# OverLordGoldDragon/ssqueezepy

Measured on AMD Instinct MI355X. Metric: ssq_cwt transforms/sec (N=160k, 300 scales, f32), higher is better.
Workload: dtype f32; 1 GPU; ssq_cwt('gmw'), N=160000, 300 log scales (nv=32), float32, two-chirp+noise; algo=blockzoom+tiles, tile_kernel=float64 tile, unordered ds_add_f64, column pair per lane (tile3_kernel)

## Files before the change

ssqueezepy_amd/csrc/ssq_blocks.h:

```cpp
#pragma once
#include "ssq_common.h"
#include "ssq_fft.h"
#include "ssq_tiles.h"
#include <algorithm>
#include <vector>

namespace ssq {

struct BlockRowDev {
    int32_t cls;
    int32_t klo;
    int32_t KP;
    int32_t L;
    int32_t G;
    int32_t pb_off;
};

struct BlockClassDev {
    int64_t P, m, V, nb;
    int64_t ctw_off;
    int64_t xb_off;
    int64_t blk_off;
    int64_t xb_stride;
    int64_t analytic;
};

struct BlockPlan {
    int64_t M = 0, N = 0, n1 = 0, na = 0, max_batch = 1;
    int dtype = SSQ_F32;
    int group = 1;
    int ncu = 256;
    int nc = 0;
    DeviceArena mem;
    std::vector<BlockClassDev> hcls;
    BlockClassDev* classes = nullptr;
    BlockRowDev* rows = nullptr;
    void* pbank = nullptr;
    void* pxi = nullptr;
    void* ctw = nullptr; void* ftw = nullptr;
    void* items[5] = {nullptr, nullptr, nullptr, nullptr, nullptr};
    std::vector<int32_t> h_items[5];
    int64_t n_items[5] = {0, 0, 0, 0, 0};
    int64_t ftw_off[5] = {0, 0, 0, 0, 0};
    void* blocks = nullptr;
    void* xb = nullptr;
    std::vector<FftPlan> ffts;
    std::vector<int> fft_first;
    void* xa = nullptr;
    FftPlan inv_m;
    AnalyticFft* ana = nullptr;
    int n_analytic = 0;
    bool own4096 = false;
    bool own_big = false;
    bool paired = true;
    int64_t n_generic = 0;
    bool exact_ok = false;
    int exA = 0, exB = 0, n_exact = 0;
    void* twM = nullptr; void* zbuf = nullptr;
    const float* e_bank = nullptr; const int64_t* e_off = nullptr; const int32_t* e_lo = nullptr;
    const int32_t* e_rows = nullptr;
    int setup_exact(const float* bank_dev, const int64_t* band_off_dev, const int32_t* band_lo_dev,
                    const int32_t* gen_rows_dev, const std::vector<int64_t>& h_off,
                    const std::vector<int32_t>& h_lo, const std::vector<int32_t>& h_gen);
    int run_exact(int sig, int nsig, const void* xh_all, float* Wx, float* dWx, float* w, unsigned short* kidx,
                  const float* row_scale, double dt, const SsqParams& sp, hipStream_t stream);

    int create(const ssq_cwt_blocks_desc& d, int dtype, int64_t M, int64_t N, int64_t n1, int64_t na,
               int64_t max_batch);
    void destroy();
    int64_t bytes() const;
    int spectra(const void* xp, const void* xh, int64_t batch, hipStream_t stream,
                const unsigned char* need = nullptr);
    int run(int sig, int nsig, float* Wx, float* dWx, float* w, unsigned short* kidx,
            const float* row_scale, double dt, const SsqParams& sp, hipStream_t stream,
            const int64_t* limit = nullptr);
    int run64(int sig, int nsig, double* Wx, double* dWx, double* w, unsigned short* kidx,
              const double* row_scale, double dt, const SsqParams& sp, hipStream_t stream);
};

}
```

ssqueezepy_amd/csrc/ssq_cwt_blocks.hip:

```cpp
#include "ssq_common.h"
#include "ssq_blocks.h"
#include "ssq_ldsfft.h"
#include <cmath>

namespace ssq {

#include "ssq_point_math.inl"

struct EmitRow {
    float2* W; float2* D; float* w; unsigned short* k;
    float rs; bool scale; double gamma; int64_t omax;
    float m2hi, m2lo;
    int fx, fa;
};
__device__ __forceinline__ EmitRow make_emit_row(float* Wx, float* dWx, float* w, unsigned short* kidx,
                                                 const float* row_scale, int sig, int ksig, int row,
                                                 int64_t na, int64_t N, double gamma, int flipud) {
    EmitRow e;
    const int64_t base = ((int64_t)sig * na + row) * N;
    e.W = reinterpret_cast<float2*>(Wx) + base;
    e.D = dWx ? reinterpret_cast<float2*>(dWx) + base : nullptr;
    e.w = w ? w + base : nullptr;
    e.k = kidx ? kidx + (int64_t)ksig * na * N + kidx_index(row, 0, na, N) : nullptr;
    e.scale = row_scale != nullptr;
// ... 2 lines not shown
    const float g2 = (float)(gamma * gamma);
    e.m2hi = g2 * 1.000004f; e.m2lo = g2 * 0.999996f;
    e.fx = flipud ? -1 : 0; e.fa = flipud ? (int)na : 0;
    return e;
}
template <bool LEAN, int GRID>
__device__ __forceinline__ bool emit_point(const EmitRow& e, int j, c32 W, c32 D, const SsqParams& sp) {
    float c = W.x, d = W.y, a = D.x, b = D.y;
    if constexpr (LEAN) {
        e.W[(unsigned)j] = make_float2(c, d);
        const float m2 = c * c + d * d, num = b * c - a * d;
        const bool above = m2 > e.m2hi, below = m2 < e.m2lo;
        const float w32 = fabsf(num * __builtin_amdgcn_rcpf(m2 * 6.2831855f));
        bool ok;
        const int kb = bin_screen_cwt<GRID>(w32, sp, (int)e.omax, ok);
        const int kf = (kb ^ e.fx) + e.fa;
        e.k[(unsigned)j] = (unsigned short)(above ? kf : 0xFFFF);
        return !(below | (above & ok));
    } else {
        c = c * e.rs; d = d * e.rs; a = a * e.rs; b = b * e.rs;
        e.W[j] = make_float2(c, d);
        if (e.D) e.D[j] = make_float2(a, b);
        if (e.w) {
            float wv;
            if (mag_lt(c, d, (float)e.gamma)) wv = INFINITY;
            else wv = (float)fabs(phase_ratio(a, b, c, d));
            e.w[j] = wv;
        }
        if (e.k) {
            const int above = mag_gt_screen(c, d, e.gamma);
            if (above < 0) return true;
            unsigned short kk = 0xFFFFu;
            if (above) {
                const int kb = bin_of_point_screen(a, b, c, d, sp, (int)e.omax);
                if (kb == -2) return true;
                kk = (unsigned short)(sp.flipud ? (int)e.omax - kb : kb);
            }
            e.k[j] = kk;
        }
        return false;
    }
}
template <int V> struct GridTag { static constexpr int value = V; };
template <bool LEAN, typename F>
__device__ __forceinline__ void dispatch_grid(int grid, F&& f) {
    if constexpr (LEAN) {
        if (grid == SSQ_GRID_LOG) f(GridTag<SSQ_GRID_LOG>{});
        else if (grid == SSQ_GRID_LOG_PIECEWISE) f(GridTag<SSQ_GRID_LOG_PIECEWISE>{});
        else f(GridTag<SSQ_GRID_LIN>{});
    } else {
        f(GridTag<-1>{});
    }
}
__device__ __forceinline__ void emit_point_exact(const EmitRow& e, unsigned short* kout, c32 W, c32 D,
                                                 const SsqParams& sp) {
    const float c = W.x * e.rs, d = W.y * e.rs, a = D.x * e.rs, b = D.y * e.rs;
    unsigned short kk = 0xFFFFu;
    if (mag_of(c, d) > e.gamma) {
        const int64_t kb = bin_of_point_exact(a, b, c, d, sp, e.omax);
        kk = (unsigned short)(sp.flipud ? e.omax - kb : kb);
    }
    *kout = kk;
}
struct BlockArgs {
    const int4* items;
    const BlockRowDev* rows;
    const BlockClassDev* classes;
    const float* pbank;
    const float* pxi;
    const c32* ctw;
    const c32* ftw;
    const c32* xb;
    const float* row_scale;
    float* Wx; float* dWx; float* w; unsigned short* kidx;
    int64_t M, N, na, n_items;
    double h;
    float inv_dt;
    double gamma;
    int sig;
    bool lean() const { return kidx && !dWx && !w && !row_scale; }
    bool wx_alone() const { return !kidx && !dWx && !w; }
};

template <int L, bool LEAN, bool NOD = false, bool PAIRED = true>
__device__ __forceinline__ void blockzoom_body(const BlockArgs& A, const SsqParams& sp, int item_idx,
                                               c32* __restrict__ buf, c32* __restrict__ spow,
                                               c32* __restrict__ wrapf, c32* __restrict__ bandW,
                                               c32* __restrict__ bandD) {
    using S = FftShape<L>;
    constexpr int G = S::G, R1 = S::R1, RL = S::RL;
    const int tid = threadIdx.x;
    const int4 item = A.items[item_idx];
    const int row = item.x, blk = item.y, c0 = item.z;
    const BlockRowDev r = A.rows[row];
    const BlockClassDev cl = A.classes[item.w];
    const int P = (int)cl.P, Rp = P / L;
    const int sig = A.sig + (int)blockIdx.y;
    const c32* xb = A.xb + cl.xb_off + ((int64_t)sig * cl.nb + blk) * cl.xb_stride;
    const c32* ctw = A.ctw + cl.ctw_off;
    const float* psi = A.pbank + r.pb_off;
    const float* pxi = A.pxi + r.pb_off;

    constexpr bool STAGE = (L <= 512);
    const float invP = 1.0f / (float)P;
    constexpr bool EARLY = !STAGE && (R1 * G <= NT);
    float e_p[EARLY ? PPT : 1], e_m[EARLY ? PPT : 1];
    c32 e_X[EARLY ? PPT : 1], e_cw[EARLY ? PPT / R1 : 1];
    if constexpr (EARLY) {
        constexpr int NBe = PPT / R1, STR = L / R1;
        c32 st_v = {0.f, 0.f}, st_w = {0.f, 0.f};
        if (tid < R1 * G) {
            const unsigned t = (unsigned)(tid / G), col = (unsigned)(c0 + tid % G);
            st_v = ctw[(t * (unsigned)STR * col) & (unsigned)(P - 1)];
        }
        if (tid < G) st_w = ctw[(0u - (unsigned)L * (unsigned)(c0 + tid)) & (unsigned)(P - 1)];
#pragma unroll
        for (int it = 0; it < NBe; ++it) {
            const int idx = tid + it * NT, g = idx % G, u = idx / G;
            const int off0 = (u - r.klo) & (L - 1);
            e_cw[it] = ctw[((unsigned)(r.klo + off0) * (unsigned)(c0 + g)) & (unsigned)(P - 1)];
#pragma unroll
            for (int k = 0; k < R1; ++k) {
                const int off = (off0 + k * STR) & (L - 1);
                const bool in = off < r.KP;
                e_p[it * R1 + k] = in ? psi[off] : 0.f;
                e_X[it * R1 + k] = in ? xb[r.klo + off] : c32{0.f, 0.f};
                e_m[it * R1 + k] = in ? pxi[off] : 0.f;
            }
        }
        if (tid < R1 * G) spow[tid] = st_v;
        if (tid < G) wrapf[tid] = st_w;
    } else {
        constexpr int STR = L / R1;
        for (int i = tid; i < R1 * G; i += NT) {
            const unsigned t = (unsigned)(i / G), col = (unsigned)(c0 + i % G);
            spow[i] = ctw[(t * (unsigned)STR * col) & (unsigned)(P - 1)];
        }
        if (tid < G) {
            const unsigned col = (unsigned)(c0 + tid);
            wrapf[tid] = ctw[(0u - (unsigned)L * col) & (unsigned)(P - 1)];
        }
        if constexpr (STAGE) {
            for (int off = tid; off < L; off += NT) {
                c32 b = {0.f, 0.f}, d = {0.f, 0.f};
                if (off < r.KP) {
                    const float p = psi[off] * invP;
                    const c32 X = xb[r.klo + off];
                    b = {p * X.x, p * X.y};
                    const float mm = pxi[off] * A.inv_dt;
                    d = {-(b.y * mm), b.x * mm};
                }
                bandW[off] = b; bandD[off] = d;
            }
        }
    }
    __syncthreads();
    c32 zw[PPT], zd[PPT];
    {
        constexpr int NB = PPT / R1, STR = L / R1;
#pragma unroll
        for (int it = 0; it < NB; ++it) {
            const int idx = tid + it * NT, g = idx % G, u = idx / G;
            const unsigned col = (unsigned)(c0 + g);
            const int off0 = (u - r.klo) & (L - 1);
            const c32 cw0 = EARLY ? e_cw[EARLY ? it : 0] : ctw[((unsigned)(r.klo + off0) * col) & (unsigned)(P - 1)];
            const c32 wf = wrapf[g];
#pragma unroll
            for (int k = 0; k < R1; ++k) {
                const int offu = off0 + k * STR;
                const int off = offu & (L - 1);
                c32 z = {0.f, 0.f}, dz = {0.f, 0.f};
                if constexpr (STAGE) {
                    c32 cw = (k == 0) ? cw0 : cmul_v(cw0, spow[k * G + g]);
                    if (offu >= L) cw = cmul_v(cw, wf);
                    z = cmul_v(bandW[off], cw);
                    dz = cmul_v(bandD[off], cw);
                } else if (EARLY || off < r.KP) {
                    const float p = (EARLY ? e_p[EARLY ? it * R1 + k : 0] : psi[off]) * invP;
                    const c32 X = EARLY ? e_X[EARLY ? it * R1 + k : 0] : xb[r.klo + off];
                    c32 cw = (k == 0) ? cw0 : cmul_v(cw0, spow[k * G + g]);
                    if (offu >= L) cw = cmul_v(cw, wf);
                    const c32 bz = {p * X.x, p * X.y};
                    z = cmul_v(bz, cw);
                    const float mm = (EARLY ? e_m[EARLY ? it * R1 + k : 0] : pxi[off]) * A.inv_dt;
                    dz = {-(z.y * mm), z.x * mm};
                }
                zw[it * R1 + k] = z; zd[it * R1 + k] = dz;
            }
        }
    }
    if constexpr (PAIRED && !NOD) {
        lds_ifft2<L>(zw, zd, buf, A.ftw, tid);
    } else {
        lds_ifft<L, true, true>(zw, buf, A.ftw, tid);
        if constexpr (!NOD) lds_ifft<L, true>(zd, buf, A.ftw, tid);
    }

    constexpr int NB = PPT / RL, STR = L / RL;
    const EmitRow er = make_emit_row(A.Wx, A.dWx, A.w, A.kidx, A.row_scale, sig, (int)blockIdx.y, row, A.na, A.N, A.gamma, sp.flipud);
    const int m = (int)cl.m, N = (int)A.N;
    const int jbase = blk * (int)cl.V - m + c0;
    const unsigned span = (unsigned)max(0, min((int)cl.V, N - blk * (int)cl.V));
    unsigned pend = 0;
    auto emit_all = [&](auto grid_tag) {
        constexpr int GRID = decltype(grid_tag)::value;
#pragma unroll
        for (int it = 0; it < NB; ++it) {
            const int idx = tid + it * NT, g = idx % G, u = idx / G;
#pragma unroll
            for (int k = 0; k < RL; ++k) {
                const int dcol = (u + k * STR) * Rp + g + (c0 - m);
                if ((unsigned)dcol >= span) continue;
                const int j = dcol + blk * (int)cl.V;
                if constexpr (NOD) {
                    er.W[j] = make_float2(zw[it * RL + k].x * er.rs, zw[it * RL + k].y * er.rs);
                    continue;
                }
                if (emit_point<LEAN, GRID>(er, j, zw[it * RL + k], NOD ? c32{0.f, 0.f} : zd[it * RL + k], sp))
                    pend |= 1u << (it * RL + k);
            }
        }
    };
    dispatch_grid<LEAN>(sp.grid, emit_all);
    while (__builtin_amdgcn_ballot_w64(pend != 0)) {
        const unsigned low = pend & (0u - pend);
        pend ^= low;
        c32 W = {0.f, 0.f}, D = {0.f, 0.f};
        int j = 0;
#pragma unroll
        for (int it = 0; it < NB; ++it) {
            const int idx = tid + it * NT, g = idx % G, u = idx / G;
#pragma unroll
            for (int k = 0; k < RL; ++k)
                if (low == (1u << (it * RL + k))) {
                    W = zw[it * RL + k]; D = NOD ? c32{0.f, 0.f} : zd[it * RL + k]; j = jbase + (u + k * STR) * Rp + g;
                }
        }
        if (low) emit_point_exact(er, er.k + j, W, D, sp);
    }
}

template <int L, bool LEAN, bool NOD = false, bool PAIRED = true>
__global__ __launch_bounds__(NT) void blockzoom_kernel(BlockArgs A, SsqParams sp) {
    __shared__ c32 buf[(PAIRED && !NOD) ? lds_ifft2_points<L> : D_POINTS];
    __shared__ c32 spow[FftShape<L>::R1 * FftShape<L>::G];
    __shared__ c32 wrapf[FftShape<L>::G];
    __shared__ c32 bandW[(L <= 512) ? L : 1], bandD[(L <= 512) ? L : 1];
    blockzoom_body<L, LEAN, NOD, PAIRED>(A, sp, (int)blockIdx.x, buf, spow, wrapf, bandW, bandD);
}

struct BlockMultiArgs {
    BlockArgs A;
    const int4* items[5]; const c32* ftw[5];
    int first[6];
};
template <bool LEAN, bool NOD = false, bool PAIRED = true>
__global__ __launch_bounds__(NT) void blockzoom_multi_kernel(BlockMultiArgs M, SsqParams sp) {
    __shared__ c32 buf[(PAIRED && !NOD) ? lds_ifft2_points<2048> : D_POINTS];
    __shared__ c32 spow[512];
    __shared__ c32 wrapf[32];
    __shared__ c32 bandW[512], bandD[512];
    const int b = (int)blockIdx.x;
    int s = 0;
#pragma unroll
    for (int k = 1; k < 5; ++k) s += b >= M.first[k];
    BlockArgs A = M.A;
    A.items = M.items[s]; A.ftw = M.ftw[s];
    const int it = b - M.first[s];
    switch (s) {
        case 0: blockzoom_body<128, LEAN, NOD, PAIRED>(A, sp, it, buf, spow, wrapf, bandW, bandD); break;
        case 1: blockzoom_body<256, LEAN, NOD, PAIRED>(A, sp, it, buf, spow, wrapf, bandW, bandD); break;
        case 2: blockzoom_body<512, LEAN, NOD, PAIRED>(A, sp, it, buf, spow, wrapf, bandW, bandD); break;
        case 3: blockzoom_body<1024, LEAN, NOD, PAIRED>(A, sp, it, buf, spow, wrapf, bandW, bandD); break;
        default: blockzoom_body<2048, LEAN, NOD, PAIRED>(A, sp, it, buf, spow, wrapf, bandW, bandD); break;
    }
}

struct BlockArgs64 {
    const int4* items; const BlockRowDev* rows; const BlockClassDev* classes;
    const double* pbank; const double* pxi;
    const c64* ctw; const c64* ftw; const c64* xb;
    const double* row_scale;
    double* Wx; double* dWx; double* w; unsigned short* kidx;
    int64_t M, N, na, n_items;
    double inv_dt, gamma;
    int sig;
    bool wx_alone() const { return !kidx && !dWx && !w; }
};

template <int L, bool NOD = false>
__global__ __launch_bounds__(FftGeom<double>::NT) SSQ_WAVES_PER_EU(2, 2) void blockzoom_f64_kernel(BlockArgs64 A, SsqParams sp) {
    using S = FftShape<L, double>;
    constexpr int NT64 = FftGeom<double>::NT, G = S::G, R1 = S::R1, RL = S::RL;
    __shared__ c64 buf[FftGeom<double>::D];
    __shared__ c64 spow[R1 * G];
    __shared__ c64 wrapf[G];
    const int tid = threadIdx.x;
    const int4 item = A.items[blockIdx.x];
    const int row = item.x, blk = item.y, c0 = item.z;
    const BlockRowDev r = A.rows[row];
    const BlockClassDev cl = A.classes[item.w];
    const int P = (int)cl.P, Rp = P / L;
    const int sig = A.sig + (int)blockIdx.y;
    const c64* xb = A.xb + cl.xb_off + ((int64_t)sig * cl.nb + blk) * cl.xb_stride;
    const c64* ctw = A.ctw + cl.ctw_off;
    const double* psi = A.pbank + r.pb_off;
    const double* pxi = A.pxi + r.pb_off;
    const double invP = 1.0 / (double)P;
    constexpr int NBP = PPT / R1, STRP = L / R1;
    double bp[PPT], bm[PPT]; c64 bX[PPT];
#pragma unroll
    for (int it = 0; it < NBP; ++it) {
        const int u = (tid + it * NT64) / G;
        const int off0 = (u - r.klo) & (L - 1);
#pragma unroll
        for (int k = 0; k < R1; ++k) {
            const int off = (off0 + k * STRP) & (L - 1);
            const int oc = off < r.KP ? off : 0;
            bp[it * R1 + k] = psi[oc]; bX[it * R1 + k] = xb[r.klo + oc]; bm[it * R1 + k] = pxi[oc];
        }
    }
    {
        constexpr int STR = L / R1;
        for (int i = tid; i < R1 * G; i += NT64) {
            const unsigned t = (unsigned)(i / G), col = (unsigned)(c0 + i % G);
            spow[i] = ctw[(t * (unsigned)STR * col) & (unsigned)(P - 1)];
        }
        if (tid < G) {
            const unsigned col = (unsigned)(c0 + tid);
            wrapf[tid] = ctw[(0u - (unsigned)L * col) & (unsigned)(P - 1)];
        }
    }
    c64 cw0s[NBP];
#pragma unroll
    for (int it = 0; it < NBP; ++it) {
        const int idx = tid + it * NT64, g = idx % G, u = idx / G;
        const int off0 = (u - r.klo) & (L - 1);
        cw0s[it] = ctw[((unsigned)(r.klo + off0) * (unsigned)(c0 + g)) & (unsigned)(P - 1)];
    }
    __syncthreads();
    c64 zw[PPT], zd[PPT];
    {
        constexpr int NB = PPT / R1, STR = L / R1;
#pragma unroll
        for (int it = 0; it < NB; ++it) {
            const int idx = tid + it * NT64, g = idx % G, u = idx / G;
            const int off0 = (u - r.klo) & (L - 1);
            const c64 cw0 = cw0s[it];
            const c64 wf = wrapf[g];
#pragma unroll
            for (int k = 0; k < R1; ++k) {
                const int offu = off0 + k * STR, off = offu & (L - 1);
                const bool in = off < r.KP;
                const double p = bp[it * R1 + k] * invP;
                const c64 X = bX[it * R1 + k];
                const double mm = bm[it * R1 + k] * A.inv_dt;
                c64 cw = (k == 0) ? cw0 : cmul(cw0, spow[k * G + g]);
// ... 365 lines not shown
                                                   c32* __restrict__ stw) {
    constexpr int L = WIDE_L, P = L * C, NTH = 64 * CW, SL = CW / C;
    const int tid = threadIdx.x;
    const int g = tid % CW, u = tid / CW, slot = g / C, r = g % C;
    const int64_t sig = blockIdx.y, M = A.M;
    const bool ana = k.analytic != 0;
    const int nunits = ana ? (int)k.nb : ((int)k.nb + 1) / 2;
    const c32* __restrict__ tw = A.ctw + k.ctw_off;
    const c32* __restrict__ xa = A.xa + sig * M;
    const float* __restrict__ xp = A.xp + sig * M;
    const int64_t lead = A.n1 - k.m;
    const int m32 = (int)M;
    wide_stage_tw<CW, C>(stw, tw, tid);
    c32 w[PPT / C][C];
    wide_load_w<CW, C>(w, tw, tid);
    c32 z[PPT];
    {
        const int unit = b * SL + slot;
        const bool live = unit < nunits;
        const int b0 = ana ? unit : 2 * unit, b1 = b0 + 1;
        const bool two = !ana && b1 < (int)k.nb;
        int64_t o0 = (lead + (int64_t)b0 * k.V) % M; if (o0 < 0) o0 += M;
        int64_t o1 = (lead + (int64_t)b1 * k.V) % M; if (o1 < 0) o1 += M;
        const int a0 = (int)o0, a1 = (int)o1;
#pragma unroll
        for (int t = 0; t < PPT; ++t) {
            const int p = (u + t * (L / 16)) * C + r;
            int s0 = a0 + p; if (s0 >= m32) s0 -= m32;
            int s1 = a1 + p; if (s1 >= m32) s1 -= m32;
            c32 v = {0.f, 0.f};
            if (live) {
                if (ana) v = xa[s0];
                else v = {xp[s0], two ? xp[s1] : 0.f};
            }
            z[t] = v;
        }
    }
    wide_ifft<CW>(z, buf, stw, tid);
    wide_natural<CW, C>(z, buf, w, tid);
    for (int sl = 0; sl < SL; ++sl) {
        const int unit = b * SL + sl;
        if (unit >= nunits) break;
        const int b0 = ana ? unit : 2 * unit;
        const bool two = !ana && b0 + 1 < (int)k.nb;
        const c32* __restrict__ Y = buf + sl * P;
        c32* out0 = A.xb + k.xb_off + (sig * k.nb + b0) * k.xb_stride;
        if (ana) {
            for (int f = tid; f < P; f += NTH) out0[f] = Y[(P - f) & (P - 1)];
        } else {
            c32* out1 = out0 + k.xb_stride;
            for (int f = tid; f <= P / 2; f += NTH) {
                const c32 Pk = Y[f], Qk = Y[(P - f) & (P - 1)];
                out0[f] = {0.5f * (Qk.x + Pk.x), 0.5f * (Qk.y - Pk.y)};
                if (two) out1[f] = {0.5f * (Qk.y + Pk.y), 0.5f * (Pk.x - Qk.x)};
            }
        }
    }
}
template <int QMAX>
__global__ __launch_bounds__(NT * QMAX) void block_spectra_multi_kernel(BlockSpecArgs A) {
    __shared__ c32 buf[4096 * QMAX];
    __shared__ c32 stw[WIDE_L];
    int b = (int)blockIdx.x, c = 0;
    while (c + 1 < A.ncls && b >= A.first[c + 1]) ++c;
    b -= A.first[c];
    const BlockClassDev k = A.classes[A.cls[c]];
    if (k.P == A.M && k.nb == 1 && !k.analytic && A.xh) {
        const int64_t M = A.M, sig = blockIdx.y;
        int64_t o = (A.n1 - k.m) % M; if (o < 0) o += M;
        const c32* __restrict__ tw = A.ctw + k.ctw_off;
        const c32* __restrict__ xh = A.xh + sig * (M / 2 + 1);
        c32* __restrict__ out0 = A.xb + k.xb_off + sig * k.nb * k.xb_stride;
        const unsigned mask = (unsigned)M - 1u, ou = (unsigned)o;
        for (int f = (int)threadIdx.x; f <= (int)(M / 2); f += NT * QMAX)
            out0[f] = cmul_v(xh[f], tw[((unsigned)f * ou) & mask]);
        return;
    }
    if (k.P == 4096) block_spectra_wide<4 * QMAX, 4>(A, k, b, buf, stw);
    else if (k.P == 8192) block_spectra_wide<4 * QMAX, 8>(A, k, b, buf, stw);
    else if constexpr (QMAX >= 4) block_spectra_wide<4 * QMAX, 16>(A, k, b, buf, stw);
}

template <int L>
static int launch_zoom(const BlockArgs& A, const SsqParams& sp, int nsig, bool paired, hipStream_t stream) {
    if (A.n_items == 0) return 0;
    const dim3 grid((unsigned)A.n_items, (unsigned)nsig);
    if (A.wx_alone())
        hipLaunchKernelGGL((blockzoom_kernel<L, false, true>), grid, dim3(NT), 0, stream, A, sp);
    else if (A.lean() && paired)
        hipLaunchKernelGGL((blockzoom_kernel<L, true>), grid, dim3(NT), 0, stream, A, sp);
    else if (A.lean())
        hipLaunchKernelGGL((blockzoom_kernel<L, true, false, false>), grid, dim3(NT), 0, stream, A, sp);
    else if (paired)
        hipLaunchKernelGGL((blockzoom_kernel<L, false>), grid, dim3(NT), 0, stream, A, sp);
    else
        hipLaunchKernelGGL((blockzoom_kernel<L, false, false, false>), grid, dim3(NT), 0, stream, A, sp);
    SSQ_LAUNCH_CHECK();
    return 0;
}

int BlockPlan::create(const ssq_cwt_blocks_desc& d, int dtype_, int64_t M_, int64_t N_, int64_t n1_,
                      int64_t na_, int64_t max_batch_) {
    M = M_; N = N_; n1 = n1_; na = na_; max_batch = max_batch_; dtype = dtype_;
    const size_t rs = dtype == SSQ_F32 ? 4 : 8;
    nc = d.n_classes;
    hcls.resize(nc);
    int64_t xb_total = 0, blk_max = 0;
    for (int c = 0; c < nc; ++c) {
        BlockClassDev& k = hcls[c];
        k.P = d.classes[5 * c]; k.m = d.classes[5 * c + 1]; k.V = d.classes[5 * c + 2];
        k.nb = d.classes[5 * c + 3];
        k.analytic = d.classes[5 * c + 4] ? 1 : 0;
        SSQ_REQUIRE(c == 0 || hcls[c - 1].analytic <= k.analytic, "block classes: analytic classes must come last");
        k.ctw_off = d.ctw_off[c];
        k.xb_stride = k.analytic ? k.P : k.P / 2 + 1;
        k.xb_off = xb_total;
        xb_total += max_batch * k.nb * k.xb_stride;
        k.blk_off = blk_max;
        if (!k.analytic) blk_max += max_batch * k.nb * k.P;
        n_analytic += (int)k.analytic;
    }
    int rc;
    if ((rc = mem.upload(&classes, hcls.data(), sizeof(BlockClassDev) * nc))) return rc;
    static_assert(sizeof(BlockRowDev) == 6 * sizeof(int32_t), "row table layout");
    if ((rc = mem.upload(&rows, d.rows, sizeof(BlockRowDev) * na))) return rc;
    if ((rc = mem.upload(&pbank, d.pbank, rs * d.n_pbank))) return rc;
    if ((rc = mem.upload(&pxi, d.pxi, rs * d.n_pbank))) return rc;
    if ((rc = mem.upload(&ctw, d.ctw, 2 * rs * (size_t)d.ctw_off[nc]))) return rc;
    if ((rc = mem.upload(&ftw, d.ftw, 2 * rs * (size_t)d.n_ftw))) return rc;
    for (int s = 0; s < 5; ++s) {
        n_items[s] = d.n_items[s];
        ftw_off[s] = d.ftw_off[s];
        if ((rc = mem.upload(&items[s], d.items[s], sizeof(int4) * (size_t)d.n_items[s]))) return rc;
        if (d.n_items[s]) h_items[s].assign(d.items[s], d.items[s] + 4 * d.n_items[s]);
    }
    if ((rc = mem.alloc(&xb, 2 * rs * (size_t)xb_total))) return rc;
    if ((rc = mem.alloc(&blocks, rs * (size_t)blk_max))) return rc;
    for (int c = 0; c < nc;) {
        int e = c;
        int64_t nblocks = 0;
        while (e < nc && hcls[e].P == hcls[c].P && hcls[e].analytic == hcls[c].analytic)
            nblocks += max_batch * hcls[e++].nb;
        FftPlan fp;
        rc = fp.create(hcls[c].analytic ? 2 : 0, dtype, (size_t)hcls[c].P, (size_t)nblocks, 1.0);
        if (rc) { fp.destroy(); return rc; }
        ffts.push_back(fp); fft_first.push_back(c);
        c = e;
    }
    if (n_analytic) {
        if ((rc = mem.alloc(&xa, 2 * rs * (size_t)(max_batch * M)))) return rc;
        if (AnalyticFft::supports(dtype, M)) {
            ana = new AnalyticFft();
            if ((rc = ana->create(M, max_batch))) return rc;
        } else {
            rc = inv_m.create(1, dtype, (size_t)M, (size_t)max_batch, 1.0 / (double)M);
            if (rc) return rc;
        }
    }
    n_generic = d.n_generic;
    own4096 = dtype == SSQ_F32 && M > 4096 && !(getenv("SSQ_DEBUG_BLOCK_SPECTRA") && !strcmp(getenv("SSQ_DEBUG_BLOCK_SPECTRA"), "rocfft"));
    own_big = own4096 && !(getenv("SSQ_DEBUG_BLOCK_SPECTRA") && !strcmp(getenv("SSQ_DEBUG_BLOCK_SPECTRA"), "4096"));
    paired = !(getenv("SSQ_DEBUG_BLOCK_PAIRED") && atoi(getenv("SSQ_DEBUG_BLOCK_PAIRED")) == 0);
    {
        int dev = 0; hipDeviceProp_t pr;
        bool lds128 = false;
        if (hipGetDevice(&dev) == hipSuccess && hipGetDeviceProperties(&pr, dev) == hipSuccess && pr.multiProcessorCount > 0) {
            ncu = pr.multiProcessorCount;
            lds128 = (size_t)pr.maxSharedMemoryPerMultiProcessor >= 128 * 1024;
        }
        own_big = own_big && lds128;
    }
    return 0;
}

void BlockPlan::destroy() {
    for (auto& f : ffts) f.destroy();
    inv_m.destroy();
    if (ana) { ana->destroy(); delete ana; ana = nullptr; }
    mem.release();
}

int64_t BlockPlan::bytes() const {
    int64_t b = mem.bytes() + (int64_t)inv_m.work_bytes + (ana ? ana->mem.bytes() : 0);
    for (const FftPlan& f : ffts) b += (int64_t)f.work_bytes;
    return b;
}

int BlockPlan::spectra(const void* xp, const void* xh, int64_t batch, hipStream_t stream,
                       const unsigned char* need) {
    (void)batch;
    std::vector<char> run_on(ffts.size(), 1);
    int lo[2] = {nc, nc}, hi[2] = {-1, -1};
    bool any_analytic = false;
    BlockSpecArgs S;
    S.ncls = 0; S.first[0] = 0;
    int qmax = 1;
    bool prefix[2] = {true, true};
    for (size_t f = 0; f < ffts.size(); ++f) {
        const int a = fft_first[f], b = f + 1 < ffts.size() ? fft_first[f + 1] : nc;
        bool on = !need;
        for (int c = a; c < b && !on; ++c) on = need[c] != 0;
        const int kind = (int)hcls[a].analytic;
        any_analytic = any_analytic || (on && kind);
        int wanted = 0;
        int64_t group_wgs = 0;
        for (int c = a; c < b; ++c) {
            if (need && !need[c]) continue;
            ++wanted;
            group_wgs += kind ? hcls[c].nb : (hcls[c].nb + 1) / 2;
        }
        const int64_t Pg = hcls[a].P;
        bool whole = Pg == M && !kind && xh;
        for (int c = a; c < b && whole; ++c) whole = hcls[c].nb == 1;
        const bool small = own_big && M < ((int64_t)1 << 30) && group_wgs * max_batch <= 2 * (int64_t)ncu &&
                           (whole || ((Pg == 8192 || Pg == 16384) && Pg <= M));
        if (on && own4096 && prefix[kind] && (Pg == 4096 || small) && S.ncls + wanted <= 8) {
            for (int c = a; c < b; ++c) {
                if (need && !need[c]) continue;
                S.cls[S.ncls++] = c;
                const bool twist = Pg == M && hcls[c].nb == 1 && !kind && xh;
                qmax = std::max(qmax, twist ? 2 : (int)(Pg / 4096));
            }
            on = false;
        }
        run_on[f] = on;
        if (on) prefix[kind] = false;
        if (on) { lo[kind] = std::min(lo[kind], a); hi[kind] = std::max(hi[kind], b - 1); }
    }
    const size_t rs = dtype == SSQ_F32 ? 4 : 8;
    if (any_analytic) {
        SSQ_REQUIRE(xh && xa, "analytic block classes need the half spectrum");
        if (ana) {
            int rc = ana->run(xh, xa, max_batch, stream);
            if (rc) return rc;
        } else {
            dim3 ga((unsigned)std::min<int64_t>((max_batch * M + 255) / 256, 4096));
            int rc = dispatch_dtype(dtype, [&](auto t) {
                using C = cx<decltype(t)>;
                hipLaunchKernelGGL(analytic_spectrum_kernel<C>, ga, dim3(256), 0, stream, (const C*)xh, (C*)xa, M, max_batch);
                SSQ_LAUNCH_CHECK();
                return 0;
            });
            if (rc) return rc;
            rc = inv_m.execute(xa, nullptr, stream);
            if (rc) return rc;
// ... 2 lines not shown
    if (S.ncls) {
        S.xp = (const float*)xp; S.xa = (const c32*)xa; S.xb = (c32*)xb; S.xh = (const c32*)xh;
        S.classes = classes; S.ctw = (const c32*)ctw; S.M = M; S.n1 = n1;
        for (int i = 0; i < S.ncls; ++i) {
            const BlockClassDev& k = hcls[S.cls[i]];
            const int64_t units = k.analytic ? k.nb : (k.nb + 1) / 2;
            const int64_t per = std::max<int64_t>(1, qmax / (k.P / 4096));
            S.first[i + 1] = S.first[i] + (int)((units + per - 1) / per);
        }
        const dim3 sg((unsigned)S.first[S.ncls], (unsigned)max_batch);
        if (qmax == 1)
            hipLaunchKernelGGL(block_spectra4096_kernel, sg, dim3(NT), 0, stream, S);
        else if (qmax == 2)
            hipLaunchKernelGGL(block_spectra_multi_kernel<2>, sg, dim3(NT * 2), 0, stream, S);
        else
            hipLaunchKernelGGL(block_spectra_multi_kernel<4>, sg, dim3(NT * 4), 0, stream, S);
        SSQ_LAUNCH_CHECK();
    }
    for (int kind = 0; kind < 2; ++kind) {
        if (hi[kind] < lo[kind]) continue;
        int64_t most = 0;
        for (int c = lo[kind]; c <= hi[kind]; ++c) most = std::max<int64_t>(most, max_batch * hcls[c].nb * hcls[c].P);
        dim3 grid((unsigned)std::min<int64_t>((most + 255) / 256, 2048), (unsigned)(hi[kind] - lo[kind] + 1));
        const int rc = dispatch_dtype(dtype, [&](auto t) {
            using T = decltype(t);
            using C = cx<T>;
            if (kind == 0)
                hipLaunchKernelGGL((gather_blocks_kernel<T, false>), grid, dim3(256), 0, stream, (const T*)xp,
                                   (T*)blocks, classes + lo[0], M, n1, max_batch);
            else
                hipLaunchKernelGGL((gather_blocks_kernel<C, true>), grid, dim3(256), 0, stream, (const C*)xa,
                                   (C*)xb, classes + lo[1], M, n1, max_batch);
            SSQ_LAUNCH_CHECK();
            return 0;
        });
        if (rc) return rc;
    }
    for (size_t f = 0; f < ffts.size(); ++f) {
        if (!run_on[f]) continue;
        const BlockClassDev& k = hcls[fft_first[f]];
        int rc = k.analytic ? ffts[f].execute((char*)xb + (size_t)k.xb_off * 2 * rs, nullptr, stream)
                            : ffts[f].execute((char*)blocks + (size_t)k.blk_off * rs,
                                              (char*)xb + (size_t)k.xb_off * 2 * rs, stream);
        if (rc) return rc;
    }
    return 0;
}

int BlockPlan::run(int sig, int nsig, float* Wx, float* dWx, float* w, unsigned short* kidx,
                   const float* row_scale, double dt, const SsqParams& sp, hipStream_t stream,
                   const int64_t* limit) {
    BlockArgs A;
    A.rows = rows; A.classes = classes; A.pbank = (const float*)pbank; A.pxi = (const float*)pxi;
    A.ctw = (const c32*)ctw;
    A.xb = (const c32*)xb; A.row_scale = row_scale;
    A.Wx = Wx; A.dWx = dWx; A.w = w; A.kidx = kidx;
    A.M = M; A.N = N; A.na = na;
    A.h = (2.0 * 3.141592653589793) / (double)M;
    A.inv_dt = 1.0f / (float)dt;
    A.gamma = sp.gamma; A.sig = sig;
    {
        const char* fe = getenv("SSQ_DEBUG_CWT_BLOCKS_MULTI");
        const int force = fe ? atoi(fe) : -1;
        int64_t total = 0, biggest = 0; int used = 0;
        for (int s = 0; s < 5; ++s) {
            const int64_t n = limit ? limit[s] : n_items[s];
            total += n; biggest = std::max(biggest, n * nsig); used += n > 0;
        }
        const bool lean = A.lean();
        const bool multi = force >= 0 ? force != 0
                                      : (used > 1 && (lean || biggest <= 2 * (int64_t)ncu || total * nsig <= 18 * (int64_t)ncu));
        if (multi && total > 0) {
            BlockMultiArgs Mx;
            Mx.A = A; Mx.A.items = nullptr; Mx.A.n_items = total; Mx.A.ftw = nullptr;
            int acc = 0;
            for (int s = 0; s < 5; ++s) {
                Mx.items[s] = (const int4*)items[s]; Mx.ftw[s] = (const c32*)ftw + ftw_off[s];
                Mx.first[s] = acc; acc += (int)(limit ? limit[s] : n_items[s]);
            }
            Mx.first[5] = acc;
            const dim3 grid((unsigned)total, (unsigned)nsig);
            if (A.wx_alone())
                hipLaunchKernelGGL((blockzoom_multi_kernel<false, true>), grid, dim3(NT), 0, stream, Mx, sp);
            else if (lean && paired)
                hipLaunchKernelGGL((blockzoom_multi_kernel<true>), grid, dim3(NT), 0, stream, Mx, sp);
            else if (lean)
                hipLaunchKernelGGL((blockzoom_multi_kernel<true, false, false>), grid, dim3(NT), 0, stream, Mx, sp);
            else if (paired)
                hipLaunchKernelGGL((blockzoom_multi_kernel<false>), grid, dim3(NT), 0, stream, Mx, sp);
            else
                hipLaunchKernelGGL((blockzoom_multi_kernel<false, false, false>), grid, dim3(NT), 0, stream, Mx, sp);
            SSQ_LAUNCH_CHECK();
            return 0;
        }
    }
    for (int s = 0; s < 5; ++s) {
        A.items = (const int4*)items[s]; A.n_items = limit ? limit[s] : n_items[s];
        A.ftw = (const c32*)ftw + ftw_off[s];
        const int rc = fft_dispatch<128, 2048>(128 << s, [&](auto len) { return launch_zoom<decltype(len)::value>(A, sp, nsig, paired, stream); });
        if (rc) return rc;
    }
    return 0;
}


int BlockPlan::setup_exact(const float* bank_dev, const int64_t* band_off_dev, const int32_t* band_lo_dev,
                           const int32_t* gen_rows_dev, const std::vector<int64_t>& h_off,
                           const std::vector<int32_t>& h_lo, const std::vector<int32_t>& h_gen) {
    exact_ok = false;
    if (h_gen.empty()) return 0;
    const int lm = fft_slot(M, 1);
    if ((1ll << lm) != M || lm < 14 || lm > 22) return 0;
    for (int32_t i : h_gen) {
        int64_t len = h_off[i + 1] - h_off[i];
        if (h_lo[i] + len > M / 2 + 1) return 0;
    }
    exA = 1 << ((lm + 1) / 2); exB = (int)(M / exA);
    e_bank = bank_dev; e_off = band_off_dev; e_lo = band_lo_dev; e_rows = gen_rows_dev;
    n_exact = (int)h_gen.size();
    std::vector<float> tw((size_t)2 * M);
    for (int64_t q = 0; q < M; ++q) {
        double ang = 2.0 * 3.14159265358979323846 * (double)q / (double)M;
        tw[2 * q] = (float)(cos(ang) / (double)M); tw[2 * q + 1] = (float)(sin(ang) / (double)M);
    }
    int rc;
    if ((rc = mem.upload(&twM, tw.data(), 8 * (size_t)M))) return rc;
    if ((rc = mem.alloc(&zbuf, (size_t)group * n_exact * 2 * M * 8))) return rc;
    exact_ok = true;
    return 0;
}

template <int L>
static int launch_exact1(const ExactArgs& E, int n_rows, int nsig, hipStream_t stream) {
    hipLaunchKernelGGL((exact_pass1_kernel<L>), dim3((unsigned)(E.A / FftShape<L>::G), (unsigned)n_rows, (unsigned)nsig),
                       dim3(NT), 0, stream, E);
    SSQ_LAUNCH_CHECK();
    return 0;
}
template <int L>
static int launch_exact2(const ExactArgs& E, const SsqParams& sp, int n_rows, int nsig, hipStream_t stream) {
    const dim3 grid((unsigned)(E.B / FftShape<L>::G), (unsigned)n_rows, (unsigned)nsig);
    if (E.lean())
        hipLaunchKernelGGL((exact_pass2_kernel<L, true>), grid, dim3(NT), 0, stream, E, sp);
    else
        hipLaunchKernelGGL((exact_pass2_kernel<L, false>), grid, dim3(NT), 0, stream, E, sp);
    SSQ_LAUNCH_CHECK();
    return 0;
}

int BlockPlan::run_exact(int sig, int nsig, const void* xh_all, float* Wx, float* dWx, float* w,
                         unsigned short* kidx, const float* row_scale, double dt, const SsqParams& sp,
                         hipStream_t stream) {
    ExactArgs E;
    E.bank = e_bank; E.band_off = e_off; E.band_lo = e_lo; E.rows = e_rows;
    E.xh = (const c32*)xh_all; E.Z = (c32*)zbuf; E.twM = (const c32*)twM; E.row_scale = row_scale;
    E.Wx = Wx; E.dWx = dWx; E.w = w; E.kidx = kidx;
    E.M = M; E.N = N; E.na = na; E.A = exA; E.B = exB; E.n1pad = (int)n1; E.sig = sig; E.n_rows = n_exact;
    E.G2 = D_POINTS / exA;
    E.h = (2.0 * 3.141592653589793) / (double)M; E.inv_dt = 1.0f / (float)dt; E.gamma = sp.gamma;
    const int rc = fft_dispatch<128, 2048>(exB, [&](auto len) {
        E.ftw = (const c32*)ftw + ftw_off[fft_slot(decltype(len)::value, 128)];
        return launch_exact1<decltype(len)::value>(E, n_exact, nsig, stream);
    });
    if (rc) return rc;
    return fft_dispatch<128, 2048>(exA, [&](auto len) {
        E.ftw = (const c32*)ftw + ftw_off[fft_slot(decltype(len)::value, 128)];
        return launch_exact2<decltype(len)::value>(E, sp, n_exact, nsig, stream);
    });
}

}
```

ssqueezepy_amd/csrc/ssq_ldsfft.h:

```cpp
#pragma once
#include <hip/hip_runtime.h>
#include "ssq_common.h"
#include <cmath>
#include <type_traits>
#include <vector>

namespace ssq {

template <typename R> struct cx { R x, y; };
using c32 = cx<float>;
using c64 = cx<double>;

__device__ __forceinline__ float fma_(float a, float b, float c) { return __builtin_fmaf(a, b, c); }
__device__ __forceinline__ double fma_(double a, double b, double c) { return __builtin_fma(a, b, c); }

template <typename R> __device__ __forceinline__ cx<R> cmul(cx<R> a, cx<R> b) {
    return {fma_(a.x, b.x, -(a.y * b.y)), fma_(a.x, b.y, a.y * b.x)};
}
__device__ __forceinline__ cx<float> cmul_v(cx<float> a, cx<float> b) {
    ssq_f2 av, bv, dv;
    av.x = a.x; av.y = a.y; bv.x = b.x; bv.y = b.y;
    SSQ_CMUL_PK(dv, av, bv);
    return {dv.x, dv.y};
}
// ... 121 lines not shown
    if constexpr (!FRESH) __syncthreads();
    {
        constexpr int NB = PPT / R1;
#pragma unroll
        for (int it = 0; it < NB; ++it) {
            cx<R> t[R1];
#pragma unroll
            for (int k = 0; k < R1; ++k) t[k] = v[it * R1 + k];
            Dft<R1>::run(t);
            int idx = tid + it * NT, g = idx % G, u = idx / G;
#pragma unroll
            for (int k = 0; k < R1; ++k) buf[(u * R1 + k) * G + g] = t[k];
        }
    }
    cx<R> tw2[ETW ? PPT / R2 : 1][ETW ? R2 : 1];
    if constexpr (ETW) {
        constexpr int NB = PPT / R2, Ns = R1, TW = L / (Ns * R2);
#pragma unroll
        for (int it = 0; it < NB; ++it) {
            const int kk = ((tid + it * NT) / G) % Ns;
#pragma unroll
            for (int k = 1; k < R2; ++k) tw2[it][k] = ftw[kk * k * TW * TWS];
        }
    }
    __syncthreads();
    {
        constexpr int NB = PPT / R2, Ns = R1, STR = L / R2;
        cx<R> t[NB][R2];
#pragma unroll
        for (int it = 0; it < NB; ++it) {
            int idx = tid + it * NT, g = idx % G, u = idx / G;
#pragma unroll
            for (int k = 0; k < R2; ++k) t[it][k] = buf[(u + k * STR) * G + g];
        }
        if (three) __syncthreads();
#pragma unroll
        for (int it = 0; it < NB; ++it) {
            int idx = tid + it * NT, g = idx % G, u = idx / G;
            int kk = u % Ns;
            constexpr int TW = L / (Ns * R2);
#pragma unroll
            for (int k = 1; k < R2; ++k) t[it][k] = cmul_v(t[it][k], ETW ? tw2[ETW ? it : 0][ETW ? k : 0] : ftw[kk * k * TW * TWS]);
            Dft<R2>::run(t[it]);
            if (three) {
                int j0 = (u / Ns) * Ns * R2 + kk;
#pragma unroll
                for (int k = 0; k < R2; ++k) buf[(j0 + k * Ns) * G + g] = t[it][k];
            } else {
#pragma unroll
                for (int k = 0; k < R2; ++k) v[it * R2 + k] = t[it][k];
            }
        }
    }
    if constexpr (three) {
        cx<R> tw3[ETW ? PPT / R3 : 1][ETW ? R3 : 1];
        if constexpr (ETW) {
#pragma unroll
            for (int it = 0; it < PPT / R3; ++it) {
                const int kk = ((tid + it * NT) / G) % (R1 * R2);
#pragma unroll
                for (int k = 1; k < R3; ++k) tw3[it][k] = ftw[kk * k * TWS];
            }
        }
        __syncthreads();
        constexpr int NB = PPT / R3, Ns = R1 * R2, STR = L / R3;
#pragma unroll
        for (int it = 0; it < NB; ++it) {
            int idx = tid + it * NT, g = idx % G, u = idx / G;
            cx<R> t[R3];
#pragma unroll
            for (int k = 0; k < R3; ++k) t[k] = buf[(u + k * STR) * G + g];
            int kk = u % Ns;
#pragma unroll
            for (int k = 1; k < R3; ++k) t[k] = cmul_v(t[k], ETW ? tw3[ETW ? it : 0][ETW ? k : 0] : ftw[kk * k * TWS]);
            Dft<R3>::run(t);
#pragma unroll
            for (int k = 0; k < R3; ++k) v[it * R3 + k] = t[k];
        }
    }
}

constexpr int lds_ifft2_pad(int L) { return (FftGeom<float>::D / L <= 8) ? 2 : 0; }
template <int L> constexpr int lds_ifft2_points = FftGeom<float>::D + lds_ifft2_pad(L) * (FftGeom<float>::D / 32);
template <int L>
__device__ __forceinline__ void lds_ifft2(cx<float> (&vw)[PPT], cx<float> (&vd)[PPT], cx<float>* __restrict__ buf,
                                          const cx<float>* __restrict__ ftw, int tid) {
    using C = cx<float>;
    constexpr int NT = FftGeom<float>::NT, G = NT * PPT / L;
    constexpr int R1 = FftShape<L>::R1, R2 = FftShape<L>::R2, R3 = FftShape<L>::R3;
    constexpr bool three = (R3 > 1);
    constexpr int NB1 = PPT / R1, NB2 = PPT / R2, STR2 = L / R2;
    constexpr int PADE = lds_ifft2_pad(L);
    static_assert(L >= 128 && (R1 * G) % 32 == 0 && 32 % (G < 32 ? G : 32) == 0, "lds_ifft2: strides and the padding");
    auto slot = [](int i) { return i + PADE * (i >> 5); };
#define SSQ_PADDED(o) ((o) + PADE * ((o) >> 5))
    auto butterflies = [](auto rr, C (&v)[PPT], auto* tw) {
        constexpr int RR = decltype(rr)::value;
#pragma unroll
        for (int it = 0; it < PPT / RR; ++it) {
            C t[RR];
            t[0] = v[it * RR];
#pragma unroll
            for (int k = 1; k < RR; ++k) {
                if constexpr (std::is_same_v<decltype(tw), std::nullptr_t*>) t[k] = v[it * RR + k];
                else t[k] = cmul_v(v[it * RR + k], tw[it][k]);
            }
            Dft<RR>::run(t);
#pragma unroll
            for (int k = 0; k < RR; ++k) v[it * RR + k] = t[k];
        }
    };
    constexpr std::nullptr_t* none = nullptr;
    int w1[NB1], r2[NB2];
#pragma unroll
    for (int it = 0; it < NB1; ++it) { const int idx = tid + it * NT; w1[it] = slot((idx / G) * R1 * G + idx % G); }
#pragma unroll
    for (int it = 0; it < NB2; ++it) { const int idx = tid + it * NT; r2[it] = slot(idx); }
    auto put1 = [&](const C (&v)[PPT]) {
#pragma unroll
        for (int it = 0; it < NB1; ++it)
#pragma unroll
            for (int k = 0; k < R1; ++k) buf[w1[it] + SSQ_PADDED(k * G)] = v[it * R1 + k];
    };
    auto get2 = [&](C (&v)[PPT]) {
#pragma unroll
        for (int it = 0; it < NB2; ++it)
#pragma unroll
            for (int k = 0; k < R2; ++k) v[it * R2 + k] = buf[r2[it] + SSQ_PADDED(k * STR2 * G)];
    };
    butterflies(FftLen<R1>{}, vw, none);
    put1(vw);
    C tw2[NB2][R2];
#pragma unroll
    for (int it = 0; it < NB2; ++it) {
        const int kk = ((tid + it * NT) / G) % R1;
        constexpr int TW = L / (R1 * R2);
#pragma unroll
        for (int k = 1; k < R2; ++k) tw2[it][k] = ftw[kk * k * TW];
    }
    butterflies(FftLen<R1>{}, vd, none);
    __syncthreads();
    get2(vw);
    __syncthreads();
    put1(vd);
    butterflies(FftLen<R2>{}, vw, tw2);
    __syncthreads();
    get2(vd);
    if constexpr (!three) {
        butterflies(FftLen<R2>{}, vd, tw2);
    } else {
        constexpr int NB3 = PPT / R3, STR3 = L / R3;
        int w2[NB2], r3[NB3];
#pragma unroll
        for (int it = 0; it < NB2; ++it) {
            const int idx = tid + it * NT, g = idx % G, u = idx / G;
            w2[it] = slot(((u / R1) * R1 * R2 + u % R1) * G + g);
        }
#pragma unroll
        for (int it = 0; it < NB3; ++it) { const int idx = tid + it * NT; r3[it] = slot(idx); }
        auto put2 = [&](const C (&v)[PPT]) {
#pragma unroll
            for (int it = 0; it < NB2; ++it)
#pragma unroll
                for (int k = 0; k < R2; ++k) buf[w2[it] + SSQ_PADDED(k * R1 * G)] = v[it * R2 + k];
        };
        auto get3 = [&](C (&v)[PPT]) {
#pragma unroll
            for (int it = 0; it < NB3; ++it)
#pragma unroll
                for (int k = 0; k < R3; ++k) v[it * R3 + k] = buf[r3[it] + SSQ_PADDED(k * STR3 * G)];
        };
        __syncthreads();
        put2(vw);
        butterflies(FftLen<R2>{}, vd, tw2);
        C tw3[NB3][R3];
#pragma unroll
        for (int it = 0; it < NB3; ++it) {
            const int kk = ((tid + it * NT) / G) % (R1 * R2);
#pragma unroll
            for (int k = 1; k < R3; ++k) tw3[it][k] = ftw[kk * k];
        }
        __syncthreads();
        get3(vw);
        __syncthreads();
        put2(vd);
        butterflies(FftLen<R3>{}, vw, tw3);
        __syncthreads();
        get3(vd);
        butterflies(FftLen<R3>{}, vd, tw3);
    }
#undef SSQ_PADDED
}

}
```

Before: 3849 transforms/s.

## Stage the wavelet band through the paired-transform LDS buffer instead of per-point registers

For the paired blockzoom path, the product of wavelet and spectrum is now precomputed once per block into the shared FFT buffer. Large L uses packed records holding the scaled band value and the frequency multiplier, and small L reuses the buffer in place of the separate bandW/bandD arrays. The derivative comes from the record's multiplier, so per-point register arrays and the bandD loads are dropped. This frees LDS and registers, and the multi kernel gains a waves-per-EU hint for the lean case. The cost is an extra barrier in lds_ifft2 before the buffer is overwritten, plus a strided record gather instead of coalesced global loads.

```diff
diff --git a/ssqueezepy_amd/csrc/ssq_blocks.h b/ssqueezepy_amd/csrc/ssq_blocks.h
--- a/ssqueezepy_amd/csrc/ssq_blocks.h
+++ b/ssqueezepy_amd/csrc/ssq_blocks.h
@@ -53,6 +53,7 @@
     bool own4096 = false;
     bool own_big = false;
     bool paired = true;
+    bool band = true;
     int64_t n_generic = 0;
     bool exact_ok = false;
     int exA = 0, exB = 0, n_exact = 0;
diff --git a/ssqueezepy_amd/csrc/ssq_cwt_blocks.hip b/ssqueezepy_amd/csrc/ssq_cwt_blocks.hip
--- a/ssqueezepy_amd/csrc/ssq_cwt_blocks.hip
+++ b/ssqueezepy_amd/csrc/ssq_cwt_blocks.hip
@@ -108,7 +108,8 @@
     bool wx_alone() const { return !kidx && !dWx && !w; }
 };
 
-template <int L, bool LEAN, bool NOD = false, bool PAIRED = true>
+struct __align__(16) BandRec { c32 b; float mm, pad; };
+template <int L, bool LEAN, bool NOD = false, bool PAIRED = true, bool BAND = PAIRED && !NOD>
 __device__ __forceinline__ void blockzoom_body(const BlockArgs& A, const SsqParams& sp, int item_idx,
                                                c32* __restrict__ buf, c32* __restrict__ spow,
                                                c32* __restrict__ wrapf, c32* __restrict__ bandW,
@@ -127,11 +128,18 @@
     const float* psi = A.pbank + r.pb_off;
     const float* pxi = A.pxi + r.pb_off;
 
+    static_assert(!BAND || (PAIRED && !NOD), "blockzoom_body: the band goes through the paired transform's buffer");
     constexpr bool STAGE = (L <= 512);
+    constexpr bool BAND_REC = BAND && !STAGE;
+    static_assert(sizeof(BandRec) == 2 * sizeof(c32) && 2 * L <= lds_ifft2_points<L>, "either form of the band: 2 L' entries of buf");
+    BandRec* __restrict__ const rec = reinterpret_cast<BandRec*>(buf);
+    c32* const bW = BAND ? buf : bandW;
+    c32* const bD = BAND ? buf + L : bandD;
     const float invP = 1.0f / (float)P;
     constexpr bool EARLY = !STAGE && (R1 * G <= NT);
-    float e_p[EARLY ? PPT : 1], e_m[EARLY ? PPT : 1];
-    c32 e_X[EARLY ? PPT : 1], e_cw[EARLY ? PPT / R1 : 1];
+    constexpr bool PERPT = EARLY && !BAND_REC;
+    float e_p[PERPT ? PPT : 1], e_m[PERPT ? PPT : 1];
+    c32 e_X[PERPT ? PPT : 1], e_cw[EARLY ? PPT / R1 : 1];
     if constexpr (EARLY) {
         constexpr int NBe = PPT / R1, STR = L / R1;
         c32 st_v = {0.f, 0.f}, st_w = {0.f, 0.f};
@@ -145,13 +153,36 @@
             const int idx = tid + it * NT, g = idx % G, u = idx / G;
             const int off0 = (u - r.klo) & (L - 1);
             e_cw[it] = ctw[((unsigned)(r.klo + off0) * (unsigned)(c0 + g)) & (unsigned)(P - 1)];
-#pragma unroll
-            for (int k = 0; k < R1; ++k) {
-                const int off = (off0 + k * STR) & (L - 1);
+            if constexpr (PERPT) {
+#pragma unroll
+                for (int k = 0; k < R1; ++k) {
+                    const int off = (off0 + k * STR) & (L - 1);
+                    const bool in = off < r.KP;
+                    e_p[it * R1 + k] = in ? psi[off] : 0.f;
+                    e_X[it * R1 + k] = in ? xb[r.klo + off] : c32{0.f, 0.f};
+                    e_m[it * R1 + k] = in ? pxi[off] : 0.f;
+                }
+            }
+        }
+        if constexpr (BAND_REC) {
+            constexpr int NE = L / NT;
+            float s_p[NE], s_m[NE]; c32 s_X[NE];
+#pragma unroll
+            for (int i = 0; i < NE; ++i) {
+                const int off = tid + i * NT;
                 const bool in = off < r.KP;
-                e_p[it * R1 + k] = in ? psi[off] : 0.f;
-                e_X[it * R1 + k] = in ? xb[r.klo + off] : c32{0.f, 0.f};
-                e_m[it * R1 + k] = in ? pxi[off] : 0.f;
+                s_p[i] = in ? psi[off] : 0.f;
+                s_X[i] = in ? xb[r.klo + off] : c32{0.f, 0.f};
+                s_m[i] = in ? pxi[off] : 0.f;
+            }
+#pragma unroll
+            for (int i = 0; i < NE; ++i) {
+                const float p = s_p[i] * invP;
+                BandRec b;
+                b.b = {p * s_X[i].x, p * s_X[i].y};
+                b.mm = s_m[i] * A.inv_dt;
+                b.pad = 0.f;
+                rec[(r.klo + tid + i * NT) & (L - 1)] = b;
             }
         }
         if (tid < R1 * G) spow[tid] = st_v;
@@ -176,7 +207,7 @@
                     const float mm = pxi[off] * A.inv_dt;
                     d = {-(b.y * mm), b.x * mm};
                 }
-                bandW[off] = b; bandD[off] = d;
+                bW[off] = b; bD[off] = d;
             }
         }
     }
@@ -199,8 +230,14 @@
                 if constexpr (STAGE) {
                     c32 cw = (k == 0) ? cw0 : cmul_v(cw0, spow[k * G + g]);
                     if (offu >= L) cw = cmul_v(cw, wf);
-                    z = cmul_v(bandW[off], cw);
-                    dz = cmul_v(bandD[off], cw);
+                    z = cmul_v(bW[off], cw);
+                    dz = cmul_v(bD[off], cw);
+                } else if constexpr (BAND_REC) {
+                    const BandRec br = rec[u + k * STR];
+                    c32 cw = (k == 0) ? cw0 : cmul_v(cw0, spow[k * G + g]);
+                    if (offu >= L) cw = cmul_v(cw, wf);
+                    z = cmul_v(br.b, cw);
+                    dz = {-(z.y * br.mm), z.x * br.mm};
                 } else if (EARLY || off < r.KP) {
                     const float p = (EARLY ? e_p[EARLY ? it * R1 + k : 0] : psi[off]) * invP;
                     const c32 X = EARLY ? e_X[EARLY ? it * R1 + k : 0] : xb[r.klo + off];
@@ -216,7 +253,7 @@
         }
     }
     if constexpr (PAIRED && !NOD) {
-        lds_ifft2<L>(zw, zd, buf, A.ftw, tid);
+        lds_ifft2<L, !BAND>(zw, zd, buf, A.ftw, tid);
     } else {
         lds_ifft<L, true, true>(zw, buf, A.ftw, tid);
         if constexpr (!NOD) lds_ifft<L, true>(zd, buf, A.ftw, tid);
@@ -266,13 +303,13 @@
     }
 }
 
-template <int L, bool LEAN, bool NOD = false, bool PAIRED = true>
+template <int L, bool LEAN, bool NOD = false, bool PAIRED = true, bool BAND = PAIRED && !NOD>
 __global__ __launch_bounds__(NT) void blockzoom_kernel(BlockArgs A, SsqParams sp) {
-    __shared__ c32 buf[(PAIRED && !NOD) ? lds_ifft2_points<L> : D_POINTS];
+    __shared__ __align__(16) c32 buf[(PAIRED && !NOD) ? lds_ifft2_points<L> : D_POINTS];
     __shared__ c32 spow[FftShape<L>::R1 * FftShape<L>::G];
     __shared__ c32 wrapf[FftShape<L>::G];
-    __shared__ c32 bandW[(L <= 512) ? L : 1], bandD[(L <= 512) ? L : 1];
-    blockzoom_body<L, LEAN, NOD, PAIRED>(A, sp, (int)blockIdx.x, buf, spow, wrapf, bandW, bandD);
+    __shared__ c32 bandW[(L <= 512 && !BAND) ? L : 1], bandD[(L <= 512 && !BAND) ? L : 1];
+    blockzoom_body<L, LEAN, NOD, PAIRED, BAND>(A, sp, (int)blockIdx.x, buf, spow, wrapf, bandW, bandD);
 }
 
 struct BlockMultiArgs {
@@ -280,12 +317,13 @@
     const int4* items[5]; const c32* ftw[5];
     int first[6];
 };
-template <bool LEAN, bool NOD = false, bool PAIRED = true>
-__global__ __launch_bounds__(NT) void blockzoom_multi_kernel(BlockMultiArgs M, SsqParams sp) {
-    __shared__ c32 buf[(PAIRED && !NOD) ? lds_ifft2_points<2048> : D_POINTS];
+template <bool LEAN, bool NOD = false, bool PAIRED = true, bool BAND = PAIRED && !NOD>
+__global__ __launch_bounds__(NT) SSQ_WAVES_PER_EU((LEAN && BAND) ? 4 : 1, (LEAN && BAND) ? 4 : 8)
+void blockzoom_multi_kernel(BlockMultiArgs M, SsqParams sp) {
+    __shared__ __align__(16) c32 buf[(PAIRED && !NOD) ? lds_ifft2_points<2048> : D_POINTS];
     __shared__ c32 spow[512];
     __shared__ c32 wrapf[32];
-    __shared__ c32 bandW[512], bandD[512];
+    __shared__ c32 bandW[BAND ? 1 : 512], bandD[BAND ? 1 : 512];
     const int b = (int)blockIdx.x;
     int s = 0;
 #pragma unroll
@@ -294,11 +332,11 @@
     A.items = M.items[s]; A.ftw = M.ftw[s];
     const int it = b - M.first[s];
     switch (s) {
-        case 0: blockzoom_body<128, LEAN, NOD, PAIRED>(A, sp, it, buf, spow, wrapf, bandW, bandD); break;
-        case 1: blockzoom_body<256, LEAN, NOD, PAIRED>(A, sp, it, buf, spow, wrapf, bandW, bandD); break;
-        case 2: blockzoom_body<512, LEAN, NOD, PAIRED>(A, sp, it, buf, spow, wrapf, bandW, bandD); break;
-        case 3: blockzoom_body<1024, LEAN, NOD, PAIRED>(A, sp, it, buf, spow, wrapf, bandW, bandD); break;
-        default: blockzoom_body<2048, LEAN, NOD, PAIRED>(A, sp, it, buf, spow, wrapf, bandW, bandD); break;
+        case 0: blockzoom_body<128, LEAN, NOD, PAIRED, BAND>(A, sp, it, buf, spow, wrapf, bandW, bandD); break;
+        case 1: blockzoom_body<256, LEAN, NOD, PAIRED, BAND>(A, sp, it, buf, spow, wrapf, bandW, bandD); break;
+        case 2: blockzoom_body<512, LEAN, NOD, PAIRED, BAND>(A, sp, it, buf, spow, wrapf, bandW, bandD); break;
+        case 3: blockzoom_body<1024, LEAN, NOD, PAIRED, BAND>(A, sp, it, buf, spow, wrapf, bandW, bandD); break;
+        default: blockzoom_body<2048, LEAN, NOD, PAIRED, BAND>(A, sp, it, buf, spow, wrapf, bandW, bandD); break;
     }
 }
 
@@ -830,17 +868,21 @@
 }
 
 template <int L>
-static int launch_zoom(const BlockArgs& A, const SsqParams& sp, int nsig, bool paired, hipStream_t stream) {
+static int launch_zoom(const BlockArgs& A, const SsqParams& sp, int nsig, bool paired, bool band, hipStream_t stream) {
     if (A.n_items == 0) return 0;
     const dim3 grid((unsigned)A.n_items, (unsigned)nsig);
     if (A.wx_alone())
         hipLaunchKernelGGL((blockzoom_kernel<L, false, true>), grid, dim3(NT), 0, stream, A, sp);
+    else if (A.lean() && paired && band)
+        hipLaunchKernelGGL((blockzoom_kernel<L, true>), grid, dim3(NT), 0, stream, A, sp);
     else if (A.lean() && paired)
-        hipLaunchKernelGGL((blockzoom_kernel<L, true>), grid, dim3(NT), 0, stream, A, sp);
+        hipLaunchKernelGGL((blockzoom_kernel<L, true, false, true, false>), grid, dim3(NT), 0, stream, A, sp);
     else if (A.lean())
         hipLaunchKernelGGL((blockzoom_kernel<L, true, false, false>), grid, dim3(NT), 0, stream, A, sp);
+    else if (paired && band)
+        hipLaunchKernelGGL((blockzoom_kernel<L, false>), grid, dim3(NT), 0, stream, A, sp);
     else if (paired)
-        hipLaunchKernelGGL((blockzoom_kernel<L, false>), grid, dim3(NT), 0, stream, A, sp);
+        hipLaunchKernelGGL((blockzoom_kernel<L, false, false, true, false>), grid, dim3(NT), 0, stream, A, sp);
     else
         hipLaunchKernelGGL((blockzoom_kernel<L, false, false, false>), grid, dim3(NT), 0, stream, A, sp);
     SSQ_LAUNCH_CHECK();
@@ -909,6 +951,7 @@
     own4096 = dtype == SSQ_F32 && M > 4096 && !(getenv("SSQ_DEBUG_BLOCK_SPECTRA") && !strcmp(getenv("SSQ_DEBUG_BLOCK_SPECTRA"), "rocfft"));
     own_big = own4096 && !(getenv("SSQ_DEBUG_BLOCK_SPECTRA") && !strcmp(getenv("SSQ_DEBUG_BLOCK_SPECTRA"), "4096"));
     paired = !(getenv("SSQ_DEBUG_BLOCK_PAIRED") && atoi(getenv("SSQ_DEBUG_BLOCK_PAIRED")) == 0);
+    band = !(getenv("SSQ_DEBUG_BLOCK_BAND") && atoi(getenv("SSQ_DEBUG_BLOCK_BAND")) == 0);
     {
         int dev = 0; hipDeviceProp_t pr;
         bool lds128 = false;
@@ -1077,12 +1120,16 @@
             const dim3 grid((unsigned)total, (unsigned)nsig);
             if (A.wx_alone())
                 hipLaunchKernelGGL((blockzoom_multi_kernel<false, true>), grid, dim3(NT), 0, stream, Mx, sp);
+            else if (lean && paired && band)
+                hipLaunchKernelGGL((blockzoom_multi_kernel<true>), grid, dim3(NT), 0, stream, Mx, sp);
             else if (lean && paired)
-                hipLaunchKernelGGL((blockzoom_multi_kernel<true>), grid, dim3(NT), 0, stream, Mx, sp);
+                hipLaunchKernelGGL((blockzoom_multi_kernel<true, false, true, false>), grid, dim3(NT), 0, stream, Mx, sp);
             else if (lean)
                 hipLaunchKernelGGL((blockzoom_multi_kernel<true, false, false>), grid, dim3(NT), 0, stream, Mx, sp);
+            else if (paired && band)
+                hipLaunchKernelGGL((blockzoom_multi_kernel<false>), grid, dim3(NT), 0, stream, Mx, sp);
             else if (paired)
-                hipLaunchKernelGGL((blockzoom_multi_kernel<false>), grid, dim3(NT), 0, stream, Mx, sp);
+                hipLaunchKernelGGL((blockzoom_multi_kernel<false, false, true, false>), grid, dim3(NT), 0, stream, Mx, sp);
             else
                 hipLaunchKernelGGL((blockzoom_multi_kernel<false, false, false>), grid, dim3(NT), 0, stream, Mx, sp);
             SSQ_LAUNCH_CHECK();
@@ -1092,7 +1139,7 @@
     for (int s = 0; s < 5; ++s) {
         A.items = (const int4*)items[s]; A.n_items = limit ? limit[s] : n_items[s];
         A.ftw = (const c32*)ftw + ftw_off[s];
-        const int rc = fft_dispatch<128, 2048>(128 << s, [&](auto len) { return launch_zoom<decltype(len)::value>(A, sp, nsig, paired, stream); });
+        const int rc = fft_dispatch<128, 2048>(128 << s, [&](auto len) { return launch_zoom<decltype(len)::value>(A, sp, nsig, paired, band, stream); });
         if (rc) return rc;
     }
     return 0;
diff --git a/ssqueezepy_amd/csrc/ssq_ldsfft.h b/ssqueezepy_amd/csrc/ssq_ldsfft.h
--- a/ssqueezepy_amd/csrc/ssq_ldsfft.h
+++ b/ssqueezepy_amd/csrc/ssq_ldsfft.h
@@ -227,7 +227,7 @@
 
 constexpr int lds_ifft2_pad(int L) { return (FftGeom<float>::D / L <= 8) ? 2 : 0; }
 template <int L> constexpr int lds_ifft2_points = FftGeom<float>::D + lds_ifft2_pad(L) * (FftGeom<float>::D / 32);
-template <int L>
+template <int L, bool FRESH = true>
 __device__ __forceinline__ void lds_ifft2(cx<float> (&vw)[PPT], cx<float> (&vd)[PPT], cx<float>* __restrict__ buf,
                                           const cx<float>* __restrict__ ftw, int tid) {
     using C = cx<float>;
@@ -274,6 +274,7 @@
             for (int k = 0; k < R2; ++k) v[it * R2 + k] = buf[r2[it] + SSQ_PADDED(k * STR2 * G)];
     };
     butterflies(FftLen<R1>{}, vw, none);
+    if constexpr (!FRESH) __syncthreads();
     put1(vw);
     C tw2[NB2][R2];
 #pragma unroll
```

Result: faster. 3902 transforms/s (median of 6 runs) (+1.4%).
